# coreperf/rejit

Measured on AMD Instinct MI355X. Metric: GB/s text scanned (regexdna 9 patterns, 50M-line input); matches/s alongside, higher is better.
Workload: dtype u8

## Files before the change

rejit_amd/csrc/plane_count.hip:

```cpp
#include <hip/hip_runtime.h>
#include <hip/hip_ext.h>

#include <cstdlib>

#include "exact_count.h"
#include "kernels.h"
#include "short_walk.h"
#include "stream_load.h"

namespace rejit_amd {

namespace {

constexpr int kWave = 64;
constexpr uint64_t kBlock = 2048;
constexpr uint32_t kPieceB = 1024;
constexpr uint32_t kStashWords = (2048 + 16) / 4;
#ifndef RJ_PC_RING
#define RJ_PC_RING 256
#endif
constexpr uint32_t kRing = RJ_PC_RING;

__device__ __forceinline__ int lane_id() { return static_cast<int>(threadIdx.x) & (kWave - 1); }

__device__ __forceinline__ uint32_t lanes_below(uint64_t mask) {
  return __builtin_amdgcn_mbcnt_hi(static_cast<uint32_t>(mask >> 32), __builtin_amdgcn_mbcnt_lo(static_cast<uint32_t>(mask), 0u));
}

__device__ __forceinline__ uint32_t from_lane_above(uint32_t v, uint32_t last) {
  return static_cast<uint32_t>(__builtin_amdgcn_update_dpp(static_cast<int>(last), static_cast<int>(v), 0x130, 0xF, 0xF, false));
}
__device__ __forceinline__ uint32_t from_lane_below(uint32_t v, uint32_t first) {
  return static_cast<uint32_t>(__builtin_amdgcn_update_dpp(static_cast<int>(first), static_cast<int>(v), 0x138, 0xF, 0xF, false));
}

template <int CTRL, int ROW_MASK>
__device__ __forceinline__ uint32_t dpp_or_zero(uint32_t x) {
  return static_cast<uint32_t>(__builtin_amdgcn_update_dpp(0, static_cast<int>(x), CTRL, ROW_MASK, 0xF, true));
}
__device__ __forceinline__ uint32_t wave_inclusive_sum(uint32_t x) {
  x += dpp_or_zero<0x111, 0xF>(x);
  x += dpp_or_zero<0x112, 0xF>(x);
  x += dpp_or_zero<0x114, 0xF>(x);
  x += dpp_or_zero<0x118, 0xF>(x);
  x += dpp_or_zero<0x142, 0xA>(x);
  x += dpp_or_zero<0x143, 0xC>(x);
  return x;
}

struct Consts {
  uint32_t cmask;
  uint32_t shift;
};

__device__ __forceinline__ uint32_t codes4(uint32_t d, const Consts& k) { return __builtin_amdgcn_udot4(d & k.cmask, 0x40100401u, 0u, false); }

__device__ __forceinline__ uint32_t codes16(const uint4& v, const Consts& k) {
  const uint32_t s = k.shift;
  return (codes4(v.x, k) >> s) | (codes4(v.y, k) << (8 - s)) | (codes4(v.z, k) << (16 - s)) | (codes4(v.w, k) << (24 - s));
}

struct Raw {
  uint4 a, b;
};

__device__ __forceinline__ void load_block(const uint8_t* block, uint32_t lane_off, Raw& r) {
  r.a = stream_load16(block + lane_off);
  r.b = stream_load16(block + lane_off + kPieceB);
}

__device__ __forceinline__ uint32_t guarded_dword(const uint8_t* text, uint64_t n, uint64_t at) {
  uint32_t v = 0;
#pragma unroll
  for (int k = 0; k < 4; k++)
    if (at + k < n) v |= static_cast<uint32_t>(text[at + k]) << (8 * k);
  return v;
}

template <int NB>
__device__ __forceinline__ uint32_t plane_test(uint32_t ta, uint32_t tb, uint32_t ha, uint32_t hb, const PlaneCountParams& a) {
  constexpr uint32_t kEven = 0x55555555u;
  const uint32_t L = (ta & kEven) | ((tb << 1) & ~kEven);
  const uint32_t H = ((ta >> 1) & kEven) | (tb & ~kEven);
  const uint32_t Ln = (ha & kEven) | ((hb << 1) & ~kEven);
  const uint32_t Hn = ((ha >> 1) & kEven) | (hb & ~kEven);
  register uint32_t q0 asm("v48") = ~(L | H);
  register uint32_t q1 asm("v49") = L & ~H;
  register uint32_t q2 asm("v50") = ~L & H;
  register uint32_t q3 asm("v51") = L & H;
  register uint32_t n0 asm("v52") = ~(Ln | Hn);
  register uint32_t n1 asm("v53") = Ln & ~Hn;
  register uint32_t n2 asm("v54") = ~Ln & Hn;
  register uint32_t n3 asm("v55") = Ln & Hn;
  uint32_t codes = ~a.mask_bits;
  asm volatile("" : "+s"(codes));
  auto code = [&](int b, int i) { return (codes >> (16 * b + 2 * i)) & 3u; };
  uint32_t E[8][NB], Z[NB], O[NB];
#pragma unroll
  for (int half = 0; half < 2; half++) {
    if (NB == 1) {
      if (half == 0) {
      asm volatile(
          "s_set_gpr_idx_on %[c00], 0x3\n"
          "v_mov_b32 %[e00], v48\n"
          "s_set_gpr_idx_idx %[c10]\n"
          "v_alignbit_b32 %[e10], v52, v48, 2\n"
          "s_set_gpr_idx_idx %[c20]\n"
          "v_alignbit_b32 %[e20], v52, v48, 4\n"
          "s_set_gpr_idx_idx %[c30]\n"
          "v_alignbit_b32 %[e30], v52, v48, 6\n"
          "s_set_gpr_idx_off\n"
          : [e00] "=&v"(E[0][0]), [e10] "=&v"(E[1][0]), [e20] "=&v"(E[2][0]), [e30] "=&v"(E[3][0])
          : [c00] "s"(code(0, 0)), [c10] "s"(code(0, 1)), [c20] "s"(code(0, 2)), [c30] "s"(code(0, 3)), "v"(q0), "v"(q1), "v"(q2), "v"(q3), "v"(n0), "v"(n1), "v"(n2), "v"(n3));
      } else {
      asm volatile(
          "s_set_gpr_idx_on %[c40], 0x3\n"
          "v_alignbit_b32 %[e40], v52, v48, 8\n"
          "s_set_gpr_idx_idx %[c50]\n"
          "v_alignbit_b32 %[e50], v52, v48, 10\n"
          "s_set_gpr_idx_idx %[c60]\n"
          "v_alignbit_b32 %[e60], v52, v48, 12\n"
          "s_set_gpr_idx_idx %[c70]\n"
          "v_alignbit_b32 %[e70], v52, v48, 14\n"
          "s_set_gpr_idx_off\n"
          : [e40] "=&v"(E[4][0]), [e50] "=&v"(E[5][0]), [e60] "=&v"(E[6][0]), [e70] "=&v"(E[7][0])
          : [c40] "s"(code(0, 4)), [c50] "s"(code(0, 5)), [c60] "s"(code(0, 6)), [c70] "s"(code(0, 7)), "v"(q0), "v"(q1), "v"(q2), "v"(q3), "v"(n0), "v"(n1), "v"(n2), "v"(n3));
      }
    } else {
      if (half == 0) {
      asm volatile(
          "s_set_gpr_idx_on %[c00], 0x3\n"
          "v_mov_b32 %[e00], v48\n"
          "s_set_gpr_idx_idx %[c01]\n"
          "v_mov_b32 %[e01], v48\n"
          "s_set_gpr_idx_idx %[c10]\n"
          "v_alignbit_b32 %[e10], v52, v48, 2\n"
          "s_set_gpr_idx_idx %[c11]\n"
          "v_alignbit_b32 %[e11], v52, v48, 2\n"
          "s_set_gpr_idx_idx %[c20]\n"
          "v_alignbit_b32 %[e20], v52, v48, 4\n"
          "s_set_gpr_idx_idx %[c21]\n"
          "v_alignbit_b32 %[e21], v52, v48, 4\n"
          "s_set_gpr_idx_idx %[c30]\n"
          "v_alignbit_b32 %[e30], v52, v48, 6\n"
          "s_set_gpr_idx_idx %[c31]\n"
          "v_alignbit_b32 %[e31], v52, v48, 6\n"
          "s_set_gpr_idx_off\n"
          : [e00] "=&v"(E[0][0]), [e01] "=&v"(E[0][1]), [e10] "=&v"(E[1][0]), [e11] "=&v"(E[1][1]), [e20] "=&v"(E[2][0]), [e21] "=&v"(E[2][1]), [e30] "=&v"(E[3][0]), [e31] "=&v"(E[3][1])
          : [c00] "s"(code(0, 0)), [c01] "s"(code(1, 0)), [c10] "s"(code(0, 1)), [c11] "s"(code(1, 1)), [c20] "s"(code(0, 2)), [c21] "s"(code(1, 2)), [c30] "s"(code(0, 3)), [c31] "s"(code(1, 3)), "v"(q0), "v"(q1), "v"(q2), "v"(q3), "v"(n0), "v"(n1), "v"(n2), "v"(n3));
      } else {
      asm volatile(
          "s_set_gpr_idx_on %[c40], 0x3\n"
          "v_alignbit_b32 %[e40], v52, v48, 8\n"
          "s_set_gpr_idx_idx %[c41]\n"
          "v_alignbit_b32 %[e41], v52, v48, 8\n"
          "s_set_gpr_idx_idx %[c50]\n"
          "v_alignbit_b32 %[e50], v52, v48, 10\n"
          "s_set_gpr_idx_idx %[c51]\n"
          "v_alignbit_b32 %[e51], v52, v48, 10\n"
          "s_set_gpr_idx_idx %[c60]\n"
          "v_alignbit_b32 %[e60], v52, v48, 12\n"
          "s_set_gpr_idx_idx %[c61]\n"
          "v_alignbit_b32 %[e61], v52, v48, 12\n"
          "s_set_gpr_idx_idx %[c70]\n"
          "v_alignbit_b32 %[e70], v52, v48, 14\n"
          "s_set_gpr_idx_idx %[c71]\n"
          "v_alignbit_b32 %[e71], v52, v48, 14\n"
          "s_set_gpr_idx_off\n"
          : [e40] "=&v"(E[4][0]), [e41] "=&v"(E[4][1]), [e50] "=&v"(E[5][0]), [e51] "=&v"(E[5][1]), [e60] "=&v"(E[6][0]), [e61] "=&v"(E[6][1]), [e70] "=&v"(E[7][0]), [e71] "=&v"(E[7][1])
          : [c40] "s"(code(0, 4)), [c41] "s"(code(1, 4)), [c50] "s"(code(0, 5)), [c51] "s"(code(1, 5)), [c60] "s"(code(0, 6)), [c61] "s"(code(1, 6)), [c70] "s"(code(0, 7)), [c71] "s"(code(1, 7)), "v"(q0), "v"(q1), "v"(q2), "v"(q3), "v"(n0), "v"(n1), "v"(n2), "v"(n3));
      }
    }
#pragma unroll
    for (int i = 4 * half; i < 4 * half + 4; i++)
#pragma unroll
      for (int b = 0; b < NB; b++) {
        const uint32_t e = E[i][b];
        if (i == 0) {
          Z[b] = e;
        } else if (i == 1) {
          O[b] = Z[b] | e;
          Z[b] &= e;
        } else {
          O[b] = Z[b] | (O[b] & e);
          if (i < 7) Z[b] &= e;
        }
      }
  }
  return NB > 1 ? (O[0] | O[NB - 1]) : O[0];
}


struct Lens {
  uint64_t w[2];
};
static_assert(kMaxFused <= 24, "two words of twelve lengths");
__device__ __forceinline__ uint32_t len_of(const Lens& l, uint32_t p) {
  return static_cast<uint32_t>((p < 12 ? l.w[0] >> (5 * p) : l.w[1] >> (5 * (p - 12))) & 31u);
}

}

template <int NB>
struct ExactShape {
  using Args = PlaneCountParams;
  static constexpr uint32_t kFixedLen = 8;
  static constexpr bool kBlobInLds = false;
  static constexpr bool kList = false;
  static constexpr bool kCapture = true;
  __device__ static __forceinline__ const PlaneCountParams& common(const Args& g) { return g; }
  __device__ static __forceinline__ uint32_t lmax(const Args&) { return 8u; }
  __device__ static __forceinline__ uint32_t offset_of(const Args&, const uint32_t*, uint32_t) { return 0u; }
  __device__ static __forceinline__ uint32_t test(uint32_t ta, uint32_t tb, uint32_t ha, uint32_t hb, const Args& g) { return plane_test<NB>(ta, tb, ha, hb, g); }
  __device__ static __forceinline__ void classify(const Args& a, const uint32_t* table, uint64_t pos, bool have, uint32_t& mask, Lens&) {
    const bool ok = have && pos >= a.sb && pos < a.se && pos + 8 <= a.n;
    uint32_t lo = 0, hi = 0;
    if (ok) {
      __builtin_memcpy(&lo, a.text + pos, 4);
      __builtin_memcpy(&hi, a.text + pos + 4, 4);
    }
    mask = exact_classify<NB>(table, a.base_lo, a.base_hi, lo, hi);
    mask = ok ? mask : 0u;
  }
  __device__ static __forceinline__ void classify_bytes(const Args& a, const uint32_t* table, uint64_t pos, bool have, uint32_t lo, uint32_t hi, uint32_t& mask) {
    const bool ok = have && pos >= a.sb && pos < a.se && pos + 8 <= a.n;
    mask = exact_classify<NB>(table, a.base_lo, a.base_hi, lo, hi);
    mask = ok ? mask : 0u;
  }
};

template <int NB>
struct ListShape {
  using Args = PlaneListParams;
  static constexpr uint32_t kFixedLen = 8;
  static constexpr bool kBlobInLds = false;
  static constexpr bool kList = true;
  static constexpr bool kCapture = false;
  __device__ static __forceinline__ void classify_bytes(const Args&, const uint32_t*, uint64_t, bool, uint32_t, uint32_t, uint32_t& mask) { mask = 0; }
  __device__ static __forceinline__ const PlaneCountParams& common(const Args& g) { return g.c; }
  __device__ static __forceinline__ uint32_t lmax(const Args&) { return 8u; }
  __device__ static __forceinline__ uint32_t offset_of(const Args&, const uint32_t*, uint32_t) { return 0u; }
  __device__ static __forceinline__ uint32_t test(uint32_t ta, uint32_t tb, uint32_t ha, uint32_t hb, const Args& g) { return plane_test<NB>(ta, tb, ha, hb, g.c); }
  __device__ static __forceinline__ void classify(const Args&, const uint32_t*, uint64_t, bool, uint32_t& mask, Lens&) { mask = 0; }
};

namespace {

template <bool TOL>
__device__ __forceinline__ uint32_t general_test(uint32_t ta, uint32_t tb, uint32_t ha, uint32_t hb, const PlaneCountGParams& g) {
  constexpr uint32_t kEven = 0x55555555u;
  const uint32_t L = (ta & kEven) | ((tb << 1) & ~kEven);
  const uint32_t H = ((ta >> 1) & kEven) | (tb & ~kEven);
  const uint32_t Ln = (ha & kEven) | ((hb << 1) & ~kEven);
  const uint32_t Hn = ((ha >> 1) & kEven) | (hb & ~kEven);
  register uint32_t q0 asm("v48") = ~(L | H);
  register uint32_t q1 asm("v49") = L & ~H;
  register uint32_t q2 asm("v50") = ~L & H;
  register uint32_t q3 asm("v51") = L & H;
  register uint32_t q4 asm("v52") = ~0u;
  register uint32_t n0 asm("v56") = ~(Ln | Hn);
  register uint32_t n1 asm("v57") = Ln & ~Hn;
  register uint32_t n2 asm("v58") = ~Ln & Hn;
  register uint32_t n3 asm("v59") = Ln & Hn;
  register uint32_t n4 asm("v60") = ~0u;
  uint32_t c = 0;
#pragma clang loop unroll(disable)
  for (uint32_t b = 0; b < g.c.n_bases; b++) {
    const uint32_t* ix = g.idx[b];
    uint32_t e0, e1, e2, e3, e4, e5, e6, e7;
    asm volatile(
        "s_set_gpr_idx_on %[i0], 0x3\n"
        "v_mov_b32 %[e0], v48\n"
        "s_set_gpr_idx_idx %[i1]\n"
        "v_alignbit_b32 %[e1], v56, v48, 2\n"
        "s_set_gpr_idx_idx %[i2]\n"
        "v_alignbit_b32 %[e2], v56, v48, 4\n"
        "s_set_gpr_idx_idx %[i3]\n"
        "v_alignbit_b32 %[e3], v56, v48, 6\n"
        "s_set_gpr_idx_idx %[i4]\n"
        "v_alignbit_b32 %[e4], v56, v48, 8\n"
        "s_set_gpr_idx_idx %[i5]\n"
        "v_alignbit_b32 %[e5], v56, v48, 10\n"
        "s_set_gpr_idx_idx %[i6]\n"
        "v_alignbit_b32 %[e6], v56, v48, 12\n"
        "s_set_gpr_idx_idx %[i7]\n"
        "v_alignbit_b32 %[e7], v56, v48, 14\n"
        "s_set_gpr_idx_off\n"
        : [e0] "=&v"(e0), [e1] "=&v"(e1), [e2] "=&v"(e2), [e3] "=&v"(e3), [e4] "=&v"(e4), [e5] "=&v"(e5), [e6] "=&v"(e6), [e7] "=&v"(e7)
        : [i0] "s"(ix[0]), [i1] "s"(ix[1]), [i2] "s"(ix[2]), [i3] "s"(ix[3]), [i4] "s"(ix[4]), [i5] "s"(ix[5]), [i6] "s"(ix[6]), [i7] "s"(ix[7]), "v"(q0), "v"(q1), "v"(q2),
          "v"(q3), "v"(q4), "v"(n0), "v"(n1), "v"(n2), "v"(n3), "v"(n4));
    if (TOL) {
      uint32_t Z = e0, O = e0 | e1;
      Z &= e1;
      O = Z | (O & e2);
      Z &= e2;
      O = Z | (O & e3);
      Z &= e3;
      O = Z | (O & e4);
      Z &= e4;
      O = Z | (O & e5);
      Z &= e5;
      O = Z | (O & e6);
      Z &= e6;
      O = Z | (O & e7);
      c |= O;
    } else {
      const uint32_t z0 = e0 & e1 & e2, z1 = e3 & e4 & e5;
      c |= z0 & z1 & e6 & e7;
    }
  }
  return c;
}

}

template <int W, int MAXK, bool TOL>
struct GeneralShape {
  using Args = PlaneCountGParams;
  static constexpr uint32_t kFixedLen = 0;
  static constexpr bool kBlobInLds = true;
  static constexpr bool kList = false;
  static constexpr bool kCapture = false;
  __device__ static __forceinline__ void classify_bytes(const Args&, const uint32_t*, uint64_t, bool, uint32_t, uint32_t, uint32_t& mask) { mask = 0; }
  __device__ static __forceinline__ const PlaneCountParams& common(const Args& g) { return g.c; }
  __device__ static __forceinline__ uint32_t lmax(const Args& g) { return g.lmax; }
  __device__ static __forceinline__ uint32_t offset_of(const Args&, const uint32_t* blob, uint32_t p) {
    return reinterpret_cast<const ClassifyDesc*>(blob)[p].win_offset;
  }
  __device__ static __forceinline__ uint32_t test(uint32_t ta, uint32_t tb, uint32_t ha, uint32_t hb, const Args& g) { return general_test<TOL>(ta, tb, ha, hb, g); }
  __device__ static __forceinline__ void classify(const Args& g, const uint32_t* blob, uint64_t w, bool have, uint32_t& mask, Lens& lens) {
    const PlaneCountParams& a = g.c;
    const ClassifyDesc* desc = reinterpret_cast<const ClassifyDesc*>(blob);
    const uint32_t* tab = blob + g.desc_words;
    uint32_t lo = 0, hi = 0;
    if (have) {
      if (w + 8 <= a.n) {
        __builtin_memcpy(&lo, a.text + w, 4);
        __builtin_memcpy(&hi, a.text + w + 4, 4);
      } else {
        for (uint32_t q = 0; q < 8 && w + q < a.n; q++) {
          const uint32_t c = a.text[w + q];
          if (q < 4) lo |= c << (8 * q);
          else hi |= c << (8 * (q - 4));
        }
      }
    }
    uint32_t todo = 0;
    for (uint32_t p = 0; p < a.n_patterns; p++) {
      const ClassifyDesc& d = desc[p];
      const uint64_t s = w - d.win_offset;
      const bool ok = have && w >= d.win_offset && s >= a.sb && s < a.se && w + d.win_len <= a.n;
      bool win = false;
      for (uint32_t q = 0; q < d.n_windows; q++) win = win || ((((lo ^ d.v0[q]) & d.m0[q]) | ((hi ^ d.v1[q]) & d.m1[q])) == 0);
      todo |= (ok && win) ? 1u << p : 0u;
    }
    mask = 0;
    lens.w[0] = lens.w[1] = 0;
    while (__ballot(todo != 0) != 0) {
      const bool act = todo != 0;
      const uint32_t p = act ? static_cast<uint32_t>(__builtin_ctz(todo)) : 0u;
      todo &= todo - 1;
      const ClassifyDesc& d = desc[p];
      const uint32_t* t0 = tab + d.tab;
      const uint64_t s = w - d.win_offset;
      uint64_t t_lo = 0, t_hi = 0;
      if (act) rj_load16(a.text, a.n, s, &t_lo, &t_hi);
      const uint32_t avail = act ? (a.n - s < 16 ? static_cast<uint32_t>(a.n - s) : 16u) : 0u;
      uint32_t len = 0;
      bool found;
      if (W == 1 || d.n_words <= 1) found = short_longest_lds<1, MAXK>(t0, d, t_lo, t_hi, avail, &len);
      else found = short_longest_lds<W, MAXK>(t0, d, t_lo, t_hi, avail, &len);
      if (found && act && len != 0) {
        mask |= 1u << p;
        if (p < 12) lens.w[0] |= static_cast<uint64_t>(len) << (5 * p);
        else lens.w[1] |= static_cast<uint64_t>(len) << (5 * (p - 12));
      }
    }
  }
};

template <bool TOL>
struct GeneralListShape {
  using Args = PlaneListGParams;
  static constexpr uint32_t kFixedLen = 0;
  static constexpr bool kBlobInLds = false;
  static constexpr bool kList = true;
  static constexpr bool kCapture = false;
  __device__ static __forceinline__ void classify_bytes(const Args&, const uint32_t*, uint64_t, bool, uint32_t, uint32_t, uint32_t& mask) { mask = 0; }
  __device__ static __forceinline__ const PlaneCountParams& common(const Args& g) { return g.g.c; }
  __device__ static __forceinline__ uint32_t lmax(const Args& g) { return g.g.lmax; }
  __device__ static __forceinline__ uint32_t offset_of(const Args&, const uint32_t*, uint32_t) { return 0u; }
  __device__ static __forceinline__ uint32_t test(uint32_t ta, uint32_t tb, uint32_t ha, uint32_t hb, const Args& g) { return general_test<TOL>(ta, tb, ha, hb, g.g); }
  __device__ static __forceinline__ void classify(const Args&, const uint32_t*, uint64_t, bool, uint32_t& mask, Lens&) { mask = 0; }
};

namespace {

struct WaveState {
  uint32_t* ring;
  uint32_t* stash;
  uint32_t head, tail;
  uint32_t acc;
  uint32_t flags;
  uint32_t prev_rel, prev_valid;
  uint32_t* ends;
  uint64_t* list;
  uint32_t list_cap;
  uint64_t list_base;
};
constexpr uint32_t kNoEnd = 0xFFFFFFFFu;

template <bool LIST, bool CAPTURE>
__device__ __forceinline__ void push_block(WaveState& w, uint32_t hm, uint32_t rel_lane, uint32_t block_rel = 0, uint32_t slot = 0) {
  const uint64_t any = __ballot(hm != 0);
  if (any == 0) return;
  auto put = [&](uint32_t idx, uint32_t rel) {
    if (LIST) {
      if (idx < w.list_cap) w.list[idx] = w.list_base + rel;
    } else {
      w.ring[idx & (kRing - 1)] = rel;
      if (CAPTURE) {
        const uint32_t o = rel - block_rel;
        const uint32_t* sw = w.stash + slot * kStashWords + (o >> 2);
        const uint32_t s0 = sw[0], s1 = sw[1], s2 = sw[2];
        w.ring[kRing + (idx & (kRing - 1))] = __builtin_amdgcn_alignbyte(s1, s0, o & 3u);
        w.ring[2 * kRing + (idx & (kRing - 1))] = __builtin_amdgcn_alignbyte(s2, s1, o & 3u);
      }
    }
  };
  const uint32_t hm_a = hm & 0x55555555u, hm_b = hm & 0xAAAAAAAAu;
  const uint64_t several = __ballot((hm & (hm - 1)) != 0);
  if (several == 0) {
    const uint64_t any_a = __ballot(hm_a != 0);
    if (hm != 0) {
      const uint32_t bit = static_cast<uint32_t>(__builtin_ctz(hm));
      const uint32_t at = hm_a != 0 ? lanes_below(any_a) : static_cast<uint32_t>(__popcll(any_a)) + lanes_below(any & ~any_a);
      put(w.tail + at, rel_lane + (bit >> 1) + ((bit & 1u) ? kPieceB : 0u));
    }
    w.tail += static_cast<uint32_t>(__popcll(any));
    return;
  }
  const uint32_t c = __popc(hm_a) | (__popc(hm_b) << 16);
  const uint32_t inc = wave_inclusive_sum(c);
  const uint32_t tots = static_cast<uint32_t>(__builtin_amdgcn_readlane(static_cast<int>(inc), kWave - 1));
  const uint32_t tot_a = tots & 0xFFFFu, tot = tot_a + (tots >> 16);
  if (LIST || tot <= kRing) {
    const uint32_t before = inc - c;
    uint32_t idx = w.tail + (before & 0xFFFFu);
    for (uint32_t m = hm_a; m; m &= m - 1, idx++) put(idx, rel_lane + (static_cast<uint32_t>(__builtin_ctz(m)) >> 1));
    idx = w.tail + tot_a + (before >> 16);
    for (uint32_t m = hm_b; m; m &= m - 1, idx++) put(idx, rel_lane + kPieceB + (static_cast<uint32_t>(__builtin_ctz(m)) >> 1));
  }
  w.tail += tot;
}

template <class S>
__device__ __forceinline__ void classify_batch(WaveState& w, uint32_t m, const uint32_t* tab, const typename S::Args& g, uint64_t span_base) {
  const PlaneCountParams& a = S::common(g);
  const int lane = lane_id();
  const bool have = static_cast<uint32_t>(lane) < m;
  const uint32_t rel = w.ring[(w.head + static_cast<uint32_t>(lane)) & (kRing - 1)];
  uint32_t mask;
  Lens lens;
  if constexpr (S::kCapture) {
    const uint32_t lo = w.ring[kRing + ((w.head + static_cast<uint32_t>(lane)) & (kRing - 1))];
    const uint32_t hi = w.ring[2 * kRing + ((w.head + static_cast<uint32_t>(lane)) & (kRing - 1))];
    S::classify_bytes(g, tab, span_base + rel, have, lo, hi, mask);
  } else {
    S::classify(g, tab, span_base + rel, have, mask, lens);
  }
  const uint32_t before = from_lane_below(rel, w.prev_rel);
  const bool has_before = lane > 0 || w.prev_valid != 0;
  const bool close = have && has_before && (rel - before) < S::lmax(g);
  if (__ballot(close && mask != 0) != 0) {
    const uint32_t all_mask = mask;
    const uint32_t suspect = close ? all_mask : 0u;
    for (uint32_t p = 0; p < a.n_patterns; p++) {
      if (__ballot(((suspect >> p) & 1u) != 0) == 0) continue;
      const uint64_t all = __ballot(((all_mask >> p) & 1u) != 0);
      const uint32_t my_len = S::kFixedLen ? S::kFixedLen : len_of(lens, p);
      const uint32_t last_rel = w.ends[4 * p + 2], last_len = w.ends[4 * p + 3];
      uint32_t kept_end = w.ends[4 * p] == kNoEnd ? 0u : static_cast<uint32_t>(__builtin_amdgcn_readfirstlane(static_cast<int>(last_rel + last_len)));
      uint64_t kept = 0;
      for (uint64_t mm = all; mm != 0; mm &= mm - 1) {
        const int i = __builtin_ctzll(mm);
        const uint32_t wi = static_cast<uint32_t>(__builtin_amdgcn_readlane(static_cast<int>(rel), i));
        const uint32_t li = static_cast<uint32_t>(__builtin_amdgcn_readlane(static_cast<int>(my_len), i));
        if (wi >= kept_end) {
          kept |= 1ull << i;
          kept_end = wi + li;
        }
      }
      if ((((all & ~kept) >> lane) & 1ull) != 0) mask &= ~(1u << p);
    }
  }
  for (uint32_t p = 0; p < a.n_patterns; p++) {
    const uint64_t mine = __ballot(((mask >> p) & 1u) != 0);
    if (mine == 0) continue;
    if (lane == static_cast<int>(p)) w.acc += static_cast<uint32_t>(__popcll(mine));
    const int fl = __builtin_ctzll(mine), ll = 63 - __builtin_clzll(mine);
    const uint32_t my_len = S::kFixedLen ? S::kFixedLen : len_of(lens, p);
    const uint32_t first = static_cast<uint32_t>(__builtin_amdgcn_readlane(static_cast<int>(rel), fl));
    const uint32_t last = static_cast<uint32_t>(__builtin_amdgcn_readlane(static_cast<int>(rel), ll));
    const uint32_t first_len = S::kFixedLen ? S::kFixedLen : static_cast<uint32_t>(__builtin_amdgcn_readlane(static_cast<int>(my_len), fl));
    const uint32_t last_len = S::kFixedLen ? S::kFixedLen : static_cast<uint32_t>(__builtin_amdgcn_readlane(static_cast<int>(my_len), ll));
    if (lane == static_cast<int>(p)) {
      if (w.ends[4 * p] == kNoEnd) {
        w.ends[4 * p] = first;
        w.ends[4 * p + 1] = first_len;
      }
      w.ends[4 * p + 2] = last;
      w.ends[4 * p + 3] = last_len;
    }
  }
  w.prev_rel = static_cast<uint32_t>(__builtin_amdgcn_readlane(static_cast<int>(rel), static_cast<int>(m - 1)));
  w.prev_valid = 1;
  w.head += m;
}

template <class S>
__device__ __forceinline__ void check_span_start(WaveState& w, uint32_t m, const uint32_t* tab, const typename S::Args& g, uint64_t span_base) {
  const PlaneCountParams& a = S::common(g);
  const int lane = lane_id();
  const uint32_t reach = S::lmax(g) - 1u;
  const uint32_t rel = w.ring[(w.head + static_cast<uint32_t>(lane)) & (kRing - 1)];
  const bool near = static_cast<uint32_t>(lane) < m && static_cast<uint32_t>(lane) < reach && rel < reach;
  if (__ballot(near) == 0 || span_base == 0) return;
  uint32_t any[2] = {0, 0};
#pragma unroll
  for (int round = 0; round < 2; round++) {
    const uint64_t pos = round == 0 ? span_base + static_cast<uint64_t>(lane) - reach : span_base + rel;
    const bool mine = round == 0 ? (static_cast<uint32_t>(lane) < reach && span_base + static_cast<uint64_t>(lane) >= reach) : near;
    uint32_t mask;
    Lens lens;
    S::classify(g, tab, pos, mine, mask, lens);
    for (uint32_t p = 0; p < a.n_patterns; p++)
      if (__ballot(((mask >> p) & 1u) != 0) != 0) any[round] |= 1u << p;
  }
  if ((any[0] & any[1]) != 0) w.flags |= kPcConflict;
}

template <class S>
__device__ __forceinline__ void blocks_done(WaveState& w, const uint32_t* tab, const typename S::Args& g, uint64_t span_base, bool& first_batch) {
  const PlaneCountParams& a = S::common(g);
  if (w.tail - w.head > kRing) {
    w.flags |= kPcVoid;
    w.head = w.tail;
    return;
  }
  while (w.tail - w.head >= a.batch_at) {
    const uint32_t held = w.tail - w.head;
    const uint32_t m = held < 64u ? held : 64u;
    if (first_batch) check_span_start<S>(w, m, tab, g, span_base);
    first_batch = false;
    classify_batch<S>(w, m, tab, g, span_base);
  }
}

}

template <class S>
__global__ __launch_bounds__(256) void plane_count(typename S::Args g) {
  __shared__ __attribute__((aligned(16))) uint32_t table[kExactTabWords];
  extern __shared__ __attribute__((aligned(16))) uint32_t blob[];
  __shared__ uint32_t rings[4][kRing * (S::kCapture ? 3 : 1)];
  __shared__ __attribute__((aligned(16))) uint32_t stashes[4][S::kCapture ? 2 * kStashWords : 4];
  __shared__ uint32_t ends[4][4 * kExactMaxPatterns];
  __shared__ unsigned long long wave_bounds[4][kExactMaxPatterns][2];
  __shared__ uint32_t wave_counts[4][kExactMaxPatterns];
  __shared__ uint32_t wave_flags[4];
  const PlaneCountParams& a = S::common(g);
  const uint32_t* tab = S::kBlobInLds ? blob : table;
  const int lane = lane_id();
  const uint32_t wid = threadIdx.x >> 6;
  const uint32_t wave = __builtin_amdgcn_readfirstlane(static_cast<uint32_t>((static_cast<uint64_t>(blockIdx.x) * blockDim.x + threadIdx.x) >> 6));
  Consts k;
  k.shift = a.code_shift;
  k.cmask = 0x03030303u << a.code_shift;
  const uint32_t c0 = static_cast<uint32_t>(a.first_block) + wave * static_cast<uint32_t>(a.span_blocks) + (wave < a.span_extra ? wave : a.span_extra);
  const uint32_t c1 = c0 + static_cast<uint32_t>(a.span_blocks) + (wave < a.span_extra ? 1u : 0u);
  const uint32_t full = static_cast<uint32_t>(a.n / kBlock);
  uint32_t fast_end = full >= 1 ? full - 1 : 0;
  if (fast_end > c1) fast_end = c1;
  if (fast_end < c0) fast_end = c0;
  const uint64_t span_base = static_cast<uint64_t>(c0) * kBlock;
  WaveState w;
  w.ring = rings[wid];
  w.stash = stashes[wid];
  w.ends = ends[wid];
  w.head = w.tail = 0;
  w.acc = 0;
  w.flags = 0;
  w.prev_rel = w.prev_valid = 0;
  w.ends[lane] = kNoEnd;
  w.ends[lane + 64] = kNoEnd;
  w.list = nullptr;
  w.list_cap = 0;
  w.list_base = 0;
  if constexpr (S::kList) {
    if (wave == 0 && lane < kCntSize)
      for (uint32_t p = 0; p < g.n_zero; p++) g.zero_counters[p][lane] = 0;
    w.list = g.hits + static_cast<uint64_t>(wave) * g.region_cap;
    w.list_cap = g.region_cap;
    w.list_base = span_base - g.offset;
  }
  bool first_batch = true;

  const uint32_t last_own = fast_end > c0 ? fast_end - 1 : c0;
  auto blk = [&](uint32_t c) { return a.text + static_cast<uint64_t>(c < last_own ? c : last_own) * kBlock; };
  const uint32_t lane_rel = static_cast<uint32_t>(lane) * 16u;
  Raw ra, rb;
  uint2 behind{0, 0};
  uint32_t c = c0;
  auto stash_put = [&](uint32_t ci, const Raw& r) __attribute__((always_inline)) {
    if constexpr (S::kCapture) {
      uint32_t* sl = w.stash + (ci & 1u) * kStashWords;
      *reinterpret_cast<uint4*>(sl + lane * 4) = r.a;
      *reinterpret_cast<uint4*>(sl + kPieceB / 4 + lane * 4) = r.b;
    }
  };
  auto spill_put = [&](uint32_t ci, uint32_t x, uint32_t y) __attribute__((always_inline)) {
    if constexpr (S::kCapture) {
      if (lane == 0) *reinterpret_cast<uint2*>(w.stash + (ci & 1u) * kStashWords + kBlock / 4) = make_uint2(x, y);
    }
  };
  if (c < fast_end) {
    load_block(blk(c), lane_rel, ra);
    load_block(blk(c + 1), lane_rel, rb);
    behind = *reinterpret_cast<const uint2*>(a.text + static_cast<uint64_t>(fast_end) * kBlock);
  }
  if (S::kList) {
  } else if (S::kBlobInLds) {
    const uint4* src = reinterpret_cast<const uint4*>(a.table);
    uint4* dst = reinterpret_cast<uint4*>(blob);
    for (uint32_t i = threadIdx.x; i < a.table_words / 4; i += blockDim.x) dst[i] = src[i];
  } else {
    for (uint32_t i = threadIdx.x; i < kExactTabWords; i += blockDim.x) table[i] = a.table[i];
  }
  __syncthreads();
  if (c < fast_end) {
    uint32_t xa = codes16(ra.a, k), xb = codes16(ra.b, k);
    stash_put(c, ra);
    if (S::kCapture) __builtin_amdgcn_sched_barrier(0);
    load_block(blk(c + 2), lane_rel, ra);
    const uint32_t behind_codes = (codes4(behind.x, k) >> k.shift) | (codes4(behind.y, k) << (8 - k.shift));
    while (c + 1 < fast_end) {
      const uint32_t ya = codes16(rb.a, k), yb = codes16(rb.b, k);
      asm volatile("" ::"v"(ya), "v"(yb));
      stash_put(c + 1, rb);
      spill_put(c, rb.a.x, rb.a.y);
      if (S::kCapture) __builtin_amdgcn_sched_barrier(0);
      if (c + 3 <= last_own) load_block(blk(c + 3), lane_rel, rb);
      {
        const uint32_t ha = from_lane_above(xa, static_cast<uint32_t>(__builtin_amdgcn_readfirstlane(static_cast<int>(xb))));
        const uint32_t hb = from_lane_above(xb, static_cast<uint32_t>(__builtin_amdgcn_readfirstlane(static_cast<int>(ya))));
        const uint32_t hm = S::test(xa, xb, ha, hb, g);
        push_block<S::kList, S::kCapture>(w, hm, (c - c0) * static_cast<uint32_t>(kBlock) + lane_rel, (c - c0) * static_cast<uint32_t>(kBlock), c & 1u);
      }
      __builtin_amdgcn_sched_barrier(0);
      xa = codes16(ra.a, k);
      xb = codes16(ra.b, k);
      asm volatile("" ::"v"(xa), "v"(xb));
      if (c + 2 < fast_end) {
        stash_put(c + 2, ra);
        spill_put(c + 1, ra.a.x, ra.a.y);
      } else {
        spill_put(c + 1, behind.x, behind.y);
      }
      if (S::kCapture) __builtin_amdgcn_sched_barrier(0);
      if (c + 4 <= last_own) load_block(blk(c + 4), lane_rel, ra);
      {
        const uint32_t next0 = c + 2 == fast_end ? behind_codes : static_cast<uint32_t>(__builtin_amdgcn_readfirstlane(static_cast<int>(xa)));
        const uint32_t ha = from_lane_above(ya, static_cast<uint32_t>(__builtin_amdgcn_readfirstlane(static_cast<int>(yb))));
        const uint32_t hb = from_lane_above(yb, next0);
        const uint32_t hm = S::test(ya, yb, ha, hb, g);
        push_block<S::kList, S::kCapture>(w, hm, (c + 1 - c0) * static_cast<uint32_t>(kBlock) + lane_rel, (c + 1 - c0) * static_cast<uint32_t>(kBlock), (c + 1) & 1u);
      }
      __builtin_amdgcn_sched_barrier(0);
      c += 2;
      if (!S::kList && w.tail - w.head >= a.batch_at) blocks_done<S>(w, tab, g, span_base, first_batch);
    }
    if (c + 1 == fast_end) {
      const uint32_t ha = from_lane_above(xa, static_cast<uint32_t>(__builtin_amdgcn_readfirstlane(static_cast<int>(xb))));
      const uint32_t hb = from_lane_above(xb, static_cast<uint32_t>(__builtin_amdgcn_readfirstlane(static_cast<int>(behind_codes))));
      const uint32_t hm = S::test(xa, xb, ha, hb, g);
      spill_put(c, behind.x, behind.y);
      push_block<S::kList, S::kCapture>(w, hm, (c - c0) * static_cast<uint32_t>(kBlock) + lane_rel, (c - c0) * static_cast<uint32_t>(kBlock), c & 1u);
      c++;
    }
    if (!S::kList) blocks_done<S>(w, tab, g, span_base, first_batch);
  }
  for (; c < c1; c++) {
    const uint64_t at = static_cast<uint64_t>(c) * kBlock + lane_rel, bt = at + kPieceB;
    uint4 va, vb;
    va.x = guarded_dword(a.text, a.n, at);
    va.y = guarded_dword(a.text, a.n, at + 4);
    va.z = guarded_dword(a.text, a.n, at + 8);
    va.w = guarded_dword(a.text, a.n, at + 12);
    vb.x = guarded_dword(a.text, a.n, bt);
    vb.y = guarded_dword(a.text, a.n, bt + 4);
    vb.z = guarded_dword(a.text, a.n, bt + 8);
    vb.w = guarded_dword(a.text, a.n, bt + 12);
    const uint32_t g0 = guarded_dword(a.text, a.n, at + 16), g1 = guarded_dword(a.text, a.n, at + 20);
    const uint32_t h0 = guarded_dword(a.text, a.n, bt + 16), h1 = guarded_dword(a.text, a.n, bt + 20);
    const uint32_t ha = (codes4(g0, k) >> k.shift) | (codes4(g1, k) << (8 - k.shift));
    const uint32_t hb = (codes4(h0, k) >> k.shift) | (codes4(h1, k) << (8 - k.shift));
    const uint32_t hm = S::test(codes16(va, k), codes16(vb, k), ha, hb, g);
    if (!S::kList && w.tail - w.head > kRing - 64u) blocks_done<S>(w, tab, g, span_base, first_batch);
    if constexpr (S::kCapture) {
      Raw gr;
      gr.a = va;
      gr.b = vb;
      stash_put(c, gr);
      const uint64_t nb = (static_cast<uint64_t>(c) + 1) * kBlock;
      spill_put(c, guarded_dword(a.text, a.n, nb), guarded_dword(a.text, a.n, nb + 4));
    }
    push_block<S::kList, S::kCapture>(w, hm, (c - c0) * static_cast<uint32_t>(kBlock) + lane_rel, (c - c0) * static_cast<uint32_t>(kBlock), c & 1u);
  }
  if constexpr (S::kList) {
    if (lane == 0) g.hit_counts[wave] = w.tail;
    return;
  }
  if (w.tail - w.head > kRing) {
    w.flags |= kPcVoid;
    w.head = w.tail;
  }
  while (w.tail != w.head) {
    const uint32_t held = w.tail - w.head;
    const uint32_t m = held < 64u ? held : 64u;
    if (first_batch) check_span_start<S>(w, m, tab, g, span_base);
    first_batch = false;
    classify_batch<S>(w, m, tab, g, span_base);
  }
  if (lane < kExactMaxPatterns) {
    const bool real = lane < static_cast<int>(a.n_patterns);
    wave_counts[wid][lane] = real ? w.acc : 0u;
    const uint32_t ef = w.ends[4 * lane], efl = w.ends[4 * lane + 1], el = w.ends[4 * lane + 2], ell = w.ends[4 * lane + 3];
    const uint64_t off = real ? S::offset_of(g, tab, static_cast<uint32_t>(lane)) : 0u;
    wave_bounds[wid][lane][0] = ef != kNoEnd ? ((span_base + ef - off) | (static_cast<unsigned long long>(efl) << kPcLenShift)) : kPcNone;
    wave_bounds[wid][lane][1] = ef != kNoEnd ? ((span_base + el - off) | (static_cast<unsigned long long>(ell) << kPcLenShift)) : kPcNone;
  }
  if (lane == 0) wave_flags[wid] = w.flags;
  __syncthreads();
  if (wid != 0 || lane >= kExactMaxPatterns) return;
  uint32_t v = wave_counts[0][lane] + wave_counts[1][lane] + wave_counts[2][lane] + wave_counts[3][lane];
  if (lane == kExactMaxPatterns - 1) v = wave_flags[0] | wave_flags[1] | wave_flags[2] | wave_flags[3];
  a.wg_rows[static_cast<uint64_t>(blockIdx.x) * kExactMaxPatterns + lane] = v;
  if (lane < static_cast<int>(a.n_patterns) && v != 0) {
    unsigned long long first = kPcNone, last = kPcNone;
#pragma unroll
    for (int q = 3; q >= 0; q--)
      if (wave_bounds[q][lane][0] != kPcNone) first = wave_bounds[q][lane][0];
#pragma unroll
    for (int q = 0; q < 4; q++)
      if (wave_bounds[q][lane][1] != kPcNone) last = wave_bounds[q][lane][1];
    *reinterpret_cast<ulonglong2*>(a.wg_bounds + (static_cast<uint64_t>(blockIdx.x) * kExactMaxPatterns + lane) * 2) = ulonglong2{first, last};
  }
}

constexpr uint32_t kFinishBatch = 8;
__global__ __launch_bounds__(256, 8) void plane_count_finish(PlaneCountParams a, uint32_t n_wg) {
  __shared__ unsigned long long part[32][kExactMaxPatterns];
  __shared__ uint32_t part_first[32][kExactMaxPatterns], part_last[32][kExactMaxPatterns];
  __shared__ uint32_t is_last;
  const uint32_t p4 = threadIdx.x & 7u, q = threadIdx.x >> 3;
  const uint32_t per = (n_wg + gridDim.x - 1) / gridDim.x;
  const uint32_t r_lo = blockIdx.x * per, r_hi = r_lo + per < n_wg ? r_lo + per : n_wg;
  uint32_t sum[4] = {0, 0, 0, 0};
  uint32_t first_row[4] = {0, 0, 0, 0}, last_row[4] = {0, 0, 0, 0};
  const uint4* rows = reinterpret_cast<const uint4*>(a.wg_rows);
  for (uint32_t r = r_lo + q; r < r_hi; r += 32 * kFinishBatch) {
    uint4 v[kFinishBatch];
#pragma unroll
    for (uint32_t i = 0; i < kFinishBatch; i++) {
      const uint32_t rr = r + 32 * i;
      v[i] = rows[static_cast<uint64_t>(rr < r_hi ? rr : r) * 8 + p4];
      if (rr >= r_hi) v[i] = uint4{0, 0, 0, 0};
    }
#pragma unroll
    for (uint32_t i = 0; i < kFinishBatch; i++) {
      const uint32_t rr1 = r + 32 * i + 1;
      const uint32_t c[4] = {v[i].x, v[i].y, v[i].z, v[i].w};
      sum[0] += v[i].x;
      sum[1] += v[i].y;
      sum[2] += v[i].z;
      sum[3] = p4 == 7 ? (sum[3] | v[i].w) : (sum[3] + v[i].w);
#pragma unroll
      for (int k = 0; k < 4; k++) {
        first_row[k] = (c[k] != 0 && first_row[k] == 0) ? rr1 : first_row[k];
        last_row[k] = c[k] != 0 ? rr1 : last_row[k];
      }
    }
  }
#pragma unroll
  for (int i = 0; i < 4; i++) {
    part[q][4 * p4 + i] = sum[i];
    part_first[q][4 * p4 + i] = first_row[i];
    part_last[q][4 * p4 + i] = last_row[i];
  }
  __syncthreads();
  const uint32_t lane = threadIdx.x & 63u, wave_id = threadIdx.x >> 6;
  if (wave_id == 0) {
    if (lane < kExactMaxPatterns) {
      unsigned long long t = 0;
      uint32_t f = 0, l = 0;
#pragma unroll 4
      for (uint32_t i = 0; i < 32; i++) {
        t = lane == kExactMaxPatterns - 1 ? (t | part[i][lane]) : (t + part[i][lane]);
        const uint32_t pf = part_first[i][lane], pl = part_last[i][lane];
        f = pf != 0 && (f == 0 || pf < f) ? pf : f;
        l = pl > l ? pl : l;
      }
      unsigned long long* g = a.acc + kPcGroupRows + blockIdx.x * 96;
      __hip_atomic_store(&g[lane], t, __ATOMIC_RELAXED, __HIP_MEMORY_SCOPE_AGENT);
      __hip_atomic_store(&g[32 + lane], static_cast<unsigned long long>(f), __ATOMIC_RELAXED, __HIP_MEMORY_SCOPE_AGENT);
      __hip_atomic_store(&g[64 + lane], static_cast<unsigned long long>(l), __ATOMIC_RELAXED, __HIP_MEMORY_SCOPE_AGENT);
    }
    if (lane == 0) {
      const unsigned long long t = __hip_atomic_fetch_add(&a.acc[kPcTicket], 1ull, __ATOMIC_ACQ_REL, __HIP_MEMORY_SCOPE_AGENT);
      is_last = t + 1 == gridDim.x ? 1u : 0u;
      if (t + 1 == gridDim.x) __hip_atomic_store(&a.acc[kPcTicket], 0ull, __ATOMIC_RELAXED, __HIP_MEMORY_SCOPE_AGENT);
    }
  }
  __syncthreads();
  if (!is_last || threadIdx.x >= kExactMaxPatterns) return;
  const uint32_t p = threadIdx.x;
  unsigned long long total = 0;
  uint32_t f = 0, l = 0;
#pragma unroll 2
  for (uint32_t g = 0; g < gridDim.x; g++) {
    const unsigned long long* row = a.acc + kPcGroupRows + g * 96;
    const unsigned long long v = __hip_atomic_load(&row[p], __ATOMIC_RELAXED, __HIP_MEMORY_SCOPE_AGENT);
    const uint32_t pf = static_cast<uint32_t>(__hip_atomic_load(&row[32 + p], __ATOMIC_RELAXED, __HIP_MEMORY_SCOPE_AGENT));
    const uint32_t pl = static_cast<uint32_t>(__hip_atomic_load(&row[64 + p], __ATOMIC_RELAXED, __HIP_MEMORY_SCOPE_AGENT));
    total = p == kExactMaxPatterns - 1 ? (total | v) : (total + v);
    f = pf != 0 && (f == 0 || pf < f) ? pf : f;
    l = pl > l ? pl : l;
  }
  if (p == kExactMaxPatterns - 1) a.host_out[kPcHostFlags] = total;
  if (p >= a.n_patterns) return;
  unsigned long long first = kPcNone, last = kPcNone;
  if (total != 0 && f != 0) {
    first = a.wg_bounds[(static_cast<uint64_t>(f - 1) * kExactMaxPatterns + p) * 2];
    last = a.wg_bounds[(static_cast<uint64_t>(l - 1) * kExactMaxPatterns + p) * 2 + 1];
  }
  a.host_out[kPcHostCount + p] = total;
  a.host_out[kPcHostBounds + 2 * p] = first;
  a.host_out[kPcHostBounds + 2 * p + 1] = last;
  a.acc[kPcBounds + 2 * p] = first;
  a.acc[kPcBounds + 2 * p + 1] = last;
  a.acc[kPcTotals + p] = total;
}

__global__ void bounds_rows_counts_kernel(BoundsParams a, const unsigned long long* acc, int64_t offset, int first_round, int64_t* rows) {
  const int p = threadIdx.x;
  if (p >= a.n_lists) return;
  uint64_t n = a.count[p];
  int64_t fb = -1, fe = -1, lb = -1, le = -1;
  if (a.spans[p]) {
    const uint64_t* r = a.spans[p];
    if (n) {
      fb = static_cast<int64_t>(r[0]) + offset;
      fe = static_cast<int64_t>(r[1]) + offset;
      lb = static_cast<int64_t>(r[2 * (n - 1)]) + offset;
      le = static_cast<int64_t>(r[2 * (n - 1) + 1]) + offset;
    }
  } else {
    n = acc[kPcTotals + p];
    if (n) {
      const unsigned long long f = acc[kPcBounds + 2 * p], l = acc[kPcBounds + 2 * p + 1];
// ... 57 lines not shown
```

Before: 50240.

## Capture candidate bytes from registers instead of LDS stash, add four-deep load ring

Drops the per-wave LDS stash that held each 2KB block so that the 8 candidate bytes could be captured on a hit. Those bytes now come straight from the lane's registers plus the neighbour lane's words through DPP, and only when the block has any hit. The capture path also gets a four-buffer register pipeline (loads three blocks ahead) and precomputes the pattern codes outside the loop. This removes LDS stores on every block and frees LDS, at the cost of more VGPRs and extra select logic on hits.

Result: no change. 49820 (median of 2 runs) (-0.8%).

```diff
diff --git a/rejit_amd/csrc/plane_count.hip b/rejit_amd/csrc/plane_count.hip
--- a/rejit_amd/csrc/plane_count.hip
+++ b/rejit_amd/csrc/plane_count.hip
@@ -2,6 +2,7 @@
 #include <hip/hip_ext.h>
 
 #include <cstdlib>
+#include <type_traits>
 
 #include "exact_count.h"
 #include "kernels.h"
@@ -15,7 +16,6 @@
 constexpr int kWave = 64;
 constexpr uint64_t kBlock = 2048;
 constexpr uint32_t kPieceB = 1024;
-constexpr uint32_t kStashWords = (2048 + 16) / 4;
 #ifndef RJ_PC_RING
 #define RJ_PC_RING 256
 #endif
@@ -77,8 +77,22 @@
   return v;
 }
 
-template <int NB>
-__device__ __forceinline__ uint32_t plane_test(uint32_t ta, uint32_t tb, uint32_t ha, uint32_t hb, const PlaneCountParams& a) {
+struct Codes {
+  uint32_t c[2][8];
+};
+__device__ __forceinline__ void extract_codes(const PlaneCountParams& a, Codes& cd) {
+  uint32_t codes = ~a.mask_bits;
+#pragma unroll
+  for (int b = 0; b < 2; b++)
+#pragma unroll
+    for (int i = 0; i < 8; i++) {
+      cd.c[b][i] = (codes >> (16 * b + 2 * i)) & 3u;
+      asm volatile("" : "+s"(cd.c[b][i]));
+    }
+}
+
+template <int NB, bool PRE>
+__device__ __forceinline__ uint32_t plane_test(uint32_t ta, uint32_t tb, uint32_t ha, uint32_t hb, const PlaneCountParams& a, const Codes* pre = nullptr) {
   constexpr uint32_t kEven = 0x55555555u;
   const uint32_t L = (ta & kEven) | ((tb << 1) & ~kEven);
   const uint32_t H = ((ta >> 1) & kEven) | (tb & ~kEven);
@@ -93,8 +107,8 @@
   register uint32_t n2 asm("v54") = ~Ln & Hn;
   register uint32_t n3 asm("v55") = Ln & Hn;
   uint32_t codes = ~a.mask_bits;
-  asm volatile("" : "+s"(codes));
-  auto code = [&](int b, int i) { return (codes >> (16 * b + 2 * i)) & 3u; };
+  if (!PRE) asm volatile("" : "+s"(codes));
+  auto code = [&](int b, int i) { return PRE ? pre->c[b][i] : (codes >> (16 * b + 2 * i)) & 3u; };
   uint32_t E[8][NB], Z[NB], O[NB];
 #pragma unroll
   for (int half = 0; half < 2; half++) {
@@ -211,7 +225,8 @@
   __device__ static __forceinline__ const PlaneCountParams& common(const Args& g) { return g; }
   __device__ static __forceinline__ uint32_t lmax(const Args&) { return 8u; }
   __device__ static __forceinline__ uint32_t offset_of(const Args&, const uint32_t*, uint32_t) { return 0u; }
-  __device__ static __forceinline__ uint32_t test(uint32_t ta, uint32_t tb, uint32_t ha, uint32_t hb, const Args& g) { return plane_test<NB>(ta, tb, ha, hb, g); }
+  __device__ static __forceinline__ uint32_t test(uint32_t ta, uint32_t tb, uint32_t ha, uint32_t hb, const Args& g) { return plane_test<NB, false>(ta, tb, ha, hb, g); }
+  __device__ static __forceinline__ uint32_t test(uint32_t ta, uint32_t tb, uint32_t ha, uint32_t hb, const Args& g, const Codes& cd) { return plane_test<NB, true>(ta, tb, ha, hb, g, &cd); }
   __device__ static __forceinline__ void classify(const Args& a, const uint32_t* table, uint64_t pos, bool have, uint32_t& mask, Lens&) {
     const bool ok = have && pos >= a.sb && pos < a.se && pos + 8 <= a.n;
     uint32_t lo = 0, hi = 0;
@@ -240,7 +255,7 @@
   __device__ static __forceinline__ const PlaneCountParams& common(const Args& g) { return g.c; }
   __device__ static __forceinline__ uint32_t lmax(const Args&) { return 8u; }
   __device__ static __forceinline__ uint32_t offset_of(const Args&, const uint32_t*, uint32_t) { return 0u; }
-  __device__ static __forceinline__ uint32_t test(uint32_t ta, uint32_t tb, uint32_t ha, uint32_t hb, const Args& g) { return plane_test<NB>(ta, tb, ha, hb, g.c); }
+  __device__ static __forceinline__ uint32_t test(uint32_t ta, uint32_t tb, uint32_t ha, uint32_t hb, const Args& g) { return plane_test<NB, false>(ta, tb, ha, hb, g.c); }
   __device__ static __forceinline__ void classify(const Args&, const uint32_t*, uint64_t, bool, uint32_t& mask, Lens&) { mask = 0; }
 };
 
@@ -398,7 +413,6 @@
 
 struct WaveState {
   uint32_t* ring;
-  uint32_t* stash;
   uint32_t head, tail;
   uint32_t acc;
   uint32_t flags;
@@ -410,21 +424,45 @@
 };
 constexpr uint32_t kNoEnd = 0xFFFFFFFFu;
 
+struct Window {
+  uint4 a, b;
+  uint2 na, nb;
+  uint2 next;
+  bool own;
+};
+
+__device__ __forceinline__ void window_bytes(const Window& v, uint32_t bit, uint32_t& lo, uint32_t& hi) {
+  const bool pb = (bit & 1u) != 0;
+  const uint32_t k = bit >> 1;
+  const uint32_t s0 = pb ? v.b.x : v.a.x, s1 = pb ? v.b.y : v.a.y, s2 = pb ? v.b.z : v.a.z, s3 = pb ? v.b.w : v.a.w;
+  const uint32_t s4 = pb ? v.nb.x : v.na.x, s5 = pb ? v.nb.y : v.na.y;
+  const bool q2 = (k & 8u) != 0, q1 = (k & 4u) != 0;
+  const uint32_t u0 = q2 ? s2 : s0, u1 = q2 ? s3 : s1, u2 = q2 ? s4 : s2, u3 = q2 ? s5 : s3;
+  const uint32_t w0 = q1 ? u1 : u0, w1 = q1 ? u2 : u1, w2 = q1 ? u3 : u2;
+  lo = __builtin_amdgcn_alignbyte(w1, w0, k & 3u);
+  hi = __builtin_amdgcn_alignbyte(w2, w1, k & 3u);
+}
+
 template <bool LIST, bool CAPTURE>
-__device__ __forceinline__ void push_block(WaveState& w, uint32_t hm, uint32_t rel_lane, uint32_t block_rel = 0, uint32_t slot = 0) {
+__device__ __forceinline__ void push_block(WaveState& w, uint32_t hm, uint32_t rel_lane, Window win = Window{}) {
   const uint64_t any = __ballot(hm != 0);
   if (any == 0) return;
-  auto put = [&](uint32_t idx, uint32_t rel) {
+  if (CAPTURE && !win.own) {
+    win.na.x = from_lane_above(win.a.x, static_cast<uint32_t>(__builtin_amdgcn_readfirstlane(static_cast<int>(win.b.x))));
+    win.na.y = from_lane_above(win.a.y, static_cast<uint32_t>(__builtin_amdgcn_readfirstlane(static_cast<int>(win.b.y))));
+    win.nb.x = from_lane_above(win.b.x, win.next.x);
+    win.nb.y = from_lane_above(win.b.y, win.next.y);
+  }
+  auto put = [&](uint32_t idx, uint32_t rel, uint32_t bit) {
     if (LIST) {
       if (idx < w.list_cap) w.list[idx] = w.list_base + rel;
     } else {
       w.ring[idx & (kRing - 1)] = rel;
       if (CAPTURE) {
-        const uint32_t o = rel - block_rel;
-        const uint32_t* sw = w.stash + slot * kStashWords + (o >> 2);
-        const uint32_t s0 = sw[0], s1 = sw[1], s2 = sw[2];
-        w.ring[kRing + (idx & (kRing - 1))] = __builtin_amdgcn_alignbyte(s1, s0, o & 3u);
-        w.ring[2 * kRing + (idx & (kRing - 1))] = __builtin_amdgcn_alignbyte(s2, s1, o & 3u);
+        uint32_t lo, hi;
+        window_bytes(win, bit, lo, hi);
+        w.ring[kRing + (idx & (kRing - 1))] = lo;
+        w.ring[2 * kRing + (idx & (kRing - 1))] = hi;
       }
     }
   };
@@ -435,7 +473,7 @@
     if (hm != 0) {
       const uint32_t bit = static_cast<uint32_t>(__builtin_ctz(hm));
       const uint32_t at = hm_a != 0 ? lanes_below(any_a) : static_cast<uint32_t>(__popcll(any_a)) + lanes_below(any & ~any_a);
-      put(w.tail + at, rel_lane + (bit >> 1) + ((bit & 1u) ? kPieceB : 0u));
+      put(w.tail + at, rel_lane + (bit >> 1) + ((bit & 1u) ? kPieceB : 0u), bit);
     }
     w.tail += static_cast<uint32_t>(__popcll(any));
     return;
@@ -447,9 +485,9 @@
   if (LIST || tot <= kRing) {
     const uint32_t before = inc - c;
     uint32_t idx = w.tail + (before & 0xFFFFu);
-    for (uint32_t m = hm_a; m; m &= m - 1, idx++) put(idx, rel_lane + (static_cast<uint32_t>(__builtin_ctz(m)) >> 1));
+    for (uint32_t m = hm_a; m; m &= m - 1, idx++) put(idx, rel_lane + (static_cast<uint32_t>(__builtin_ctz(m)) >> 1), static_cast<uint32_t>(__builtin_ctz(m)));
     idx = w.tail + tot_a + (before >> 16);
-    for (uint32_t m = hm_b; m; m &= m - 1, idx++) put(idx, rel_lane + kPieceB + (static_cast<uint32_t>(__builtin_ctz(m)) >> 1));
+    for (uint32_t m = hm_b; m; m &= m - 1, idx++) put(idx, rel_lane + kPieceB + (static_cast<uint32_t>(__builtin_ctz(m)) >> 1), static_cast<uint32_t>(__builtin_ctz(m)));
   }
   w.tail += tot;
 }
@@ -564,7 +602,6 @@
   __shared__ __attribute__((aligned(16))) uint32_t table[kExactTabWords];
   extern __shared__ __attribute__((aligned(16))) uint32_t blob[];
   __shared__ uint32_t rings[4][kRing * (S::kCapture ? 3 : 1)];
-  __shared__ __attribute__((aligned(16))) uint32_t stashes[4][S::kCapture ? 2 * kStashWords : 4];
   __shared__ uint32_t ends[4][4 * kExactMaxPatterns];
   __shared__ unsigned long long wave_bounds[4][kExactMaxPatterns][2];
   __shared__ uint32_t wave_counts[4][kExactMaxPatterns];
@@ -586,7 +623,6 @@
   const uint64_t span_base = static_cast<uint64_t>(c0) * kBlock;
   WaveState w;
   w.ring = rings[wid];
-  w.stash = stashes[wid];
   w.ends = ends[wid];
   w.head = w.tail = 0;
   w.acc = 0;
@@ -609,72 +645,111 @@
   const uint32_t last_own = fast_end > c0 ? fast_end - 1 : c0;
   auto blk = [&](uint32_t c) { return a.text + static_cast<uint64_t>(c < last_own ? c : last_own) * kBlock; };
   const uint32_t lane_rel = static_cast<uint32_t>(lane) * 16u;
-  Raw ra, rb;
   uint2 behind{0, 0};
   uint32_t c = c0;
-  auto stash_put = [&](uint32_t ci, const Raw& r) __attribute__((always_inline)) {
-    if constexpr (S::kCapture) {
-      uint32_t* sl = w.stash + (ci & 1u) * kStashWords;
-      *reinterpret_cast<uint4*>(sl + lane * 4) = r.a;
-      *reinterpret_cast<uint4*>(sl + kPieceB / 4 + lane * 4) = r.b;
-    }
+  auto stage = [&]() __attribute__((always_inline)) {
+    if (S::kList) {
+    } else if (S::kBlobInLds) {
+      const uint4* src = reinterpret_cast<const uint4*>(a.table);
+      uint4* dst = reinterpret_cast<uint4*>(blob);
+      for (uint32_t i = threadIdx.x; i < a.table_words / 4; i += blockDim.x) dst[i] = src[i];
+    } else {
+      for (uint32_t i = threadIdx.x; i < kExactTabWords; i += blockDim.x) table[i] = a.table[i];
+    }
+    __syncthreads();
   };
-  auto spill_put = [&](uint32_t ci, uint32_t x, uint32_t y) __attribute__((always_inline)) {
-    if constexpr (S::kCapture) {
-      if (lane == 0) *reinterpret_cast<uint2*>(w.stash + (ci & 1u) * kStashWords + kBlock / 4) = make_uint2(x, y);
-    }
-  };
+  if constexpr (S::kCapture) {
+    Raw q0, q1, q2, q3;
+    if (c < fast_end) {
+      load_block(blk(c), lane_rel, q0);
+      load_block(blk(c + 1), lane_rel, q1);
+      load_block(blk(c + 2), lane_rel, q2);
+      behind = *reinterpret_cast<const uint2*>(a.text + static_cast<uint64_t>(fast_end) * kBlock);
+    }
+    stage();
+    if (c < fast_end) {
+      const uint32_t behind_codes = (codes4(behind.x, k) >> k.shift) | (codes4(behind.y, k) << (8 - k.shift));
+      uint32_t xa = codes16(q0.a, k), xb = codes16(q0.b, k);
+      Codes cd;
+      extract_codes(a, cd);
+      auto step = [&](auto guarded, const Raw& cur, const Raw& n1, Raw& n3) __attribute__((always_inline)) {
+        const bool last = decltype(guarded)::value && c + 1 == fast_end;
+        const uint32_t ya = codes16(n1.a, k), yb = codes16(n1.b, k);
+        asm volatile("" ::"v"(ya), "v"(yb));
+        if (!decltype(guarded)::value || c + 3 <= last_own) load_block(blk(c + 3), lane_rel, n3);
+        Window win;
+        win.a = cur.a;
+        win.b = cur.b;
+        win.own = false;
+        win.next.x = last ? behind.x : static_cast<uint32_t>(__builtin_amdgcn_readfirstlane(static_cast<int>(n1.a.x)));
+        win.next.y = last ? behind.y : static_cast<uint32_t>(__builtin_amdgcn_readfirstlane(static_cast<int>(n1.a.y)));
+        const uint32_t next0 = last ? behind_codes : static_cast<uint32_t>(__builtin_amdgcn_readfirstlane(static_cast<int>(ya)));
+        const uint32_t ha = from_lane_above(xa, static_cast<uint32_t>(__builtin_amdgcn_readfirstlane(static_cast<int>(xb))));
+        const uint32_t hb = from_lane_above(xb, next0);
+        const uint32_t hm = S::test(xa, xb, ha, hb, g, cd);
+        push_block<false, true>(w, hm, (c - c0) * static_cast<uint32_t>(kBlock) + lane_rel, win);
+        __builtin_amdgcn_sched_barrier(0);
+        xa = ya;
+        xb = yb;
+        c++;
+      };
+      using Free = std::integral_constant<bool, false>;
+      using Guarded = std::integral_constant<bool, true>;
+      while (c + 6 <= last_own) {
+        step(Free{}, q0, q1, q3);
+        step(Free{}, q1, q2, q0);
+        if (w.tail - w.head >= a.batch_at) blocks_done<S>(w, tab, g, span_base, first_batch);
+        step(Free{}, q2, q3, q1);
+        step(Free{}, q3, q0, q2);
+        if (w.tail - w.head >= a.batch_at) blocks_done<S>(w, tab, g, span_base, first_batch);
+      }
+      for (;;) {
+        step(Guarded{}, q0, q1, q3);
+        if (c >= fast_end) break;
+        step(Guarded{}, q1, q2, q0);
+        if (c >= fast_end) break;
+        if (w.tail - w.head >= a.batch_at) blocks_done<S>(w, tab, g, span_base, first_batch);
+        step(Guarded{}, q2, q3, q1);
+        if (c >= fast_end) break;
+        step(Guarded{}, q3, q0, q2);
+        if (c >= fast_end) break;
+        if (w.tail - w.head >= a.batch_at) blocks_done<S>(w, tab, g, span_base, first_batch);
+      }
+      blocks_done<S>(w, tab, g, span_base, first_batch);
+    }
+  } else {
+  Raw ra, rb;
   if (c < fast_end) {
     load_block(blk(c), lane_rel, ra);
     load_block(blk(c + 1), lane_rel, rb);
     behind = *reinterpret_cast<const uint2*>(a.text + static_cast<uint64_t>(fast_end) * kBlock);
   }
-  if (S::kList) {
-  } else if (S::kBlobInLds) {
-    const uint4* src = reinterpret_cast<const uint4*>(a.table);
-    uint4* dst = reinterpret_cast<uint4*>(blob);
-    for (uint32_t i = threadIdx.x; i < a.table_words / 4; i += blockDim.x) dst[i] = src[i];
-  } else {
-    for (uint32_t i = threadIdx.x; i < kExactTabWords; i += blockDim.x) table[i] = a.table[i];
-  }
-  __syncthreads();
+  stage();
   if (c < fast_end) {
     uint32_t xa = codes16(ra.a, k), xb = codes16(ra.b, k);
-    stash_put(c, ra);
-    if (S::kCapture) __builtin_amdgcn_sched_barrier(0);
     load_block(blk(c + 2), lane_rel, ra);
     const uint32_t behind_codes = (codes4(behind.x, k) >> k.shift) | (codes4(behind.y, k) << (8 - k.shift));
     while (c + 1 < fast_end) {
       const uint32_t ya = codes16(rb.a, k), yb = codes16(rb.b, k);
       asm volatile("" ::"v"(ya), "v"(yb));
-      stash_put(c + 1, rb);
-      spill_put(c, rb.a.x, rb.a.y);
-      if (S::kCapture) __builtin_amdgcn_sched_barrier(0);
       if (c + 3 <= last_own) load_block(blk(c + 3), lane_rel, rb);
       {
         const uint32_t ha = from_lane_above(xa, static_cast<uint32_t>(__builtin_amdgcn_readfirstlane(static_cast<int>(xb))));
         const uint32_t hb = from_lane_above(xb, static_cast<uint32_t>(__builtin_amdgcn_readfirstlane(static_cast<int>(ya))));
         const uint32_t hm = S::test(xa, xb, ha, hb, g);
-        push_block<S::kList, S::kCapture>(w, hm, (c - c0) * static_cast<uint32_t>(kBlock) + lane_rel, (c - c0) * static_cast<uint32_t>(kBlock), c & 1u);
+        push_block<S::kList, false>(w, hm, (c - c0) * static_cast<uint32_t>(kBlock) + lane_rel);
       }
       __builtin_amdgcn_sched_barrier(0);
       xa = codes16(ra.a, k);
       xb = codes16(ra.b, k);
       asm volatile("" ::"v"(xa), "v"(xb));
-      if (c + 2 < fast_end) {
-        stash_put(c + 2, ra);
-        spill_put(c + 1, ra.a.x, ra.a.y);
-      } else {
-        spill_put(c + 1, behind.x, behind.y);
-      }
-      if (S::kCapture) __builtin_amdgcn_sched_barrier(0);
       if (c + 4 <= last_own) load_block(blk(c + 4), lane_rel, ra);
       {
         const uint32_t next0 = c + 2 == fast_end ? behind_codes : static_cast<uint32_t>(__builtin_amdgcn_readfirstlane(static_cast<int>(xa)));
         const uint32_t ha = from_lane_above(ya, static_cast<uint32_t>(__builtin_amdgcn_readfirstlane(static_cast<int>(yb))));
         const uint32_t hb = from_lane_above(yb, next0);
         const uint32_t hm = S::test(ya, yb, ha, hb, g);
-        push_block<S::kList, S::kCapture>(w, hm, (c + 1 - c0) * static_cast<uint32_t>(kBlock) + lane_rel, (c + 1 - c0) * static_cast<uint32_t>(kBlock), (c + 1) & 1u);
+        push_block<S::kList, false>(w, hm, (c + 1 - c0) * static_cast<uint32_t>(kBlock) + lane_rel);
       }
       __builtin_amdgcn_sched_barrier(0);
       c += 2;
@@ -684,11 +759,11 @@
       const uint32_t ha = from_lane_above(xa, static_cast<uint32_t>(__builtin_amdgcn_readfirstlane(static_cast<int>(xb))));
       const uint32_t hb = from_lane_above(xb, static_cast<uint32_t>(__builtin_amdgcn_readfirstlane(static_cast<int>(behind_codes))));
       const uint32_t hm = S::test(xa, xb, ha, hb, g);
-      spill_put(c, behind.x, behind.y);
-      push_block<S::kList, S::kCapture>(w, hm, (c - c0) * static_cast<uint32_t>(kBlock) + lane_rel, (c - c0) * static_cast<uint32_t>(kBlock), c & 1u);
+      push_block<S::kList, false>(w, hm, (c - c0) * static_cast<uint32_t>(kBlock) + lane_rel);
       c++;
     }
     if (!S::kList) blocks_done<S>(w, tab, g, span_base, first_batch);
+  }
   }
   for (; c < c1; c++) {
     const uint64_t at = static_cast<uint64_t>(c) * kBlock + lane_rel, bt = at + kPieceB;
@@ -707,15 +782,15 @@
     const uint32_t hb = (codes4(h0, k) >> k.shift) | (codes4(h1, k) << (8 - k.shift));
     const uint32_t hm = S::test(codes16(va, k), codes16(vb, k), ha, hb, g);
     if (!S::kList && w.tail - w.head > kRing - 64u) blocks_done<S>(w, tab, g, span_base, first_batch);
+    Window win;
     if constexpr (S::kCapture) {
-      Raw gr;
-      gr.a = va;
-      gr.b = vb;
-      stash_put(c, gr);
-      const uint64_t nb = (static_cast<uint64_t>(c) + 1) * kBlock;
-      spill_put(c, guarded_dword(a.text, a.n, nb), guarded_dword(a.text, a.n, nb + 4));
-    }
-    push_block<S::kList, S::kCapture>(w, hm, (c - c0) * static_cast<uint32_t>(kBlock) + lane_rel, (c - c0) * static_cast<uint32_t>(kBlock), c & 1u);
+      win.a = va;
+      win.b = vb;
+      win.na = make_uint2(g0, g1);
+      win.nb = make_uint2(h0, h1);
+      win.own = true;
+    }
+    push_block<S::kList, S::kCapture>(w, hm, (c - c0) * static_cast<uint32_t>(kBlock) + lane_rel, win);
   }
   if constexpr (S::kList) {
     if (lane == 0) g.hit_counts[wave] = w.tail;
```
